# LPD-EPFL-ML/X-MAP

Measured on AMD Instinct MI355X. Metric: item_sim_pairs_per_s, higher is better.
Workload: dtype f64

## Files before the change

x-map_amd/csrc/common.h:

```cpp
#pragma once
#if defined(__HIP_DEVICE_COMPILE__) && !defined(__gfx950__)
#error "libxmap_hip is written for gfx950 (MI355X): build with --offload-arch=gfx950"
#endif
#include <hip/hip_runtime.h>
#include <stdint.h>
#include <stdio.h>
#include <string.h>

#include "../../include/xmap_hip.h"

namespace xmap {

void set_error(const char *fmt, ...);

#define XM_HIP(call)                                                                         \
    do {                                                                                     \
        hipError_t e_ = (call);                                                              \
        if (e_ != hipSuccess) {                                                              \
            xmap::set_error("%s:%d %s -> %s", __FILE__, __LINE__, #call, hipGetErrorString(e_)); \
            return XMAP_ERR_HIP;                                                             \
        }                                                                                    \
    } while (0)

#define XM_LAUNCH_CHECK() XM_HIP(hipGetLastError())

#define XM_ARG(cond)                                                        \
    do {                                                                    \
        if (!(cond)) {                                                      \
            xmap::set_error("%s:%d bad argument: %s", __FILE__, __LINE__, #cond); \
            return XMAP_ERR_ARG;                                            \
        }                                                                   \
    } while (0)

hipError_t xm_malloc_async(void **p, size_t bytes, hipStream_t st);
hipError_t xm_free_async(void *p, hipStream_t st);
struct XmScope {
    int dev; hipStream_t st; size_t live0; bool ok;
    explicit XmScope(hipStream_t st);
    ~XmScope();
    XmScope(const XmScope &) = delete;
    XmScope &operator=(const XmScope &) = delete;
};
#define XM_SCOPE(stream) xmap::XmScope xm_scope_((hipStream_t)(stream))
constexpr int HW_SLOTS = 2, HW_WORDS = 16;
constexpr int HW_PLAN = 0, HW_PAIRS = 1;
struct HostWait { int dev; int64_t *h; hipEvent_t ev[HW_SLOTS]; bool pending[HW_SLOTS]; };
HostWait *host_wait();
int host_wait_post(hipStream_t st, int slot, const void *d_src, int words);
int host_wait_take(int slot, const int64_t **h);
struct FillList {
    enum { MAX = 8 };
    void *p[MAX]; unsigned long long words[MAX]; unsigned val[MAX]; int n;
    FillList() : n(0) {}
    void add(void *ptr, size_t bytes, unsigned v = 0u) {
        if (n >= MAX) { n = MAX + 1; return; }
        p[n] = ptr; words[n] = bytes / 4; val[n] = v; n++;
    }
};
int fill_multi(hipStream_t st, const FillList &F);
int radix_sort_pairs(hipStream_t st, unsigned long long *keys, int *vals, unsigned long long *keys_tmp, int *vals_tmp, long long n,
                     int bits);

constexpr int WAVE = 64;

__device__ __forceinline__ int lane_id() { return threadIdx.x & 63; }

__device__ __forceinline__ int rl32(int v, int l) { return __builtin_amdgcn_readlane(v, l); }
__device__ __forceinline__ float rlf(float v, int l) { return __int_as_float(rl32(__float_as_int(v), l)); }
__device__ __forceinline__ long long rl64(long long v, int l) {
    int lo = rl32((int)(v & 0xffffffffll), l), hi = rl32((int)(v >> 32), l);
    return ((long long)hi << 32) | (unsigned int)lo;
}
__device__ __forceinline__ double rld(double v, int l) {
    return __longlong_as_double(rl64(__double_as_longlong(v), l));
}
__device__ __forceinline__ int uniform(int v) { return __builtin_amdgcn_readfirstlane(v); }

__device__ __forceinline__ unsigned long long lanemask_lt() {
    return (1ull << lane_id()) - 1ull;
}

__device__ __forceinline__ double wave_sum(double v) {
// ... 37 lines not shown
```

x-map_amd/csrc/tri.h:

```cpp
#pragma once
#include "common.h"
#include "tilesort.h"

namespace xmap {

constexpr int T_SLOTS = 1024;
constexpr int HMAX = 1024;
constexpr int SMALL_BOUND = 96;
constexpr int MID_BOUND = 384;

constexpr int N_CLASSES = 5;
constexpr int WIDE_MIN = 2048;
__host__ __device__ __forceinline__ int class_rank(int cls) {
    return cls == 4 ? 0 : (cls == 0 ? 1 : (cls == 2 ? 2 : (cls == 3 ? 3 : 4)));
}

__device__ __forceinline__ double weighted(double cs, int n, int cap) {
    const int mn = n < cap ? n : cap;
    return 1.0 * cs * (double)mn / (double)cap;
}
__device__ __forceinline__ unsigned long long ls_key(double d) {
    return (d != d) ? 0x7ff8000000000000ull : (unsigned long long)__double_as_longlong(d);
}

struct RaterRec { int e0; int pos_ge; float rating; int user; };
struct UbWide { int item_ge; int pad; double rating; };
struct RaterRecWide { int e0; int pos_ge; double rating; };

constexpr int COO_SHARDS = 4096;

int mirror_counts(hipStream_t st, int n_items, long long range_cap, int n_ranges, const unsigned long long *cur, const int *coo_i,
                  const int *coo_j, bool skip_self, int *part, int *counts, FillList *fills = nullptr);
void ts_geometry(int K, long long M, int ch, ts::Geo &G);
int ts_prepare(hipStream_t st, ts::Geo &G, const long long *ptr, FillList *fills = nullptr);
extern template __global__ void ts::k_ts_bin<3, true, ts::RecLoader<3>>(ts::Geo, ts::RecLoader<3>, long long, unsigned long long *__restrict__);

}
```

x-map_amd/csrc/tri_layout.hip:

```cpp
#include "tri.h"
#include "item_stats.h"

namespace xmap {

__device__ __forceinline__ unsigned long long wkey(int n, int item) {
    return ((unsigned long long)(unsigned)n << 32) | (unsigned)item;
}

constexpr int HIST_LDS = 2048;
constexpr int HIST_PER = 16;
__global__ __launch_bounds__(256) void k_hist(int I, const long long *iptr, int HB, int *hist) {
    __shared__ int loc[HIST_LDS];
    for (int t = threadIdx.x; t < HIST_LDS; t += 256) loc[t] = 0;
    __syncthreads();
    const long long base = (long long)blockIdx.x * 256 * HIST_PER;
    for (int q = 0; q < HIST_PER; q++) {
        const long long i = base + (long long)q * 256 + threadIdx.x;
        if (i < I) {
            long long n = iptr[i + 1] - iptr[i];
            int bin = n < HB - 1 ? (int)n : HB - 1;
            if (bin < HIST_LDS) atomicAdd(&loc[bin], 1); else atomicAdd(&hist[bin], 1);
        }
    }
    __syncthreads();
// ... 556 lines not shown
    for (long long p = p0 + lane_id(); p < p1; p += 64) {
        double r; int u;
        src.load(p, r, u);
        src.set_flag(p, r >= avg);
    }
}

__global__ __launch_bounds__(256) void k_rc_flags(long long nnz, RaterRec *rc, const int2 *ub, const double *info) {
    const long long p = (long long)blockIdx.x * blockDim.x + threadIdx.x;
    if (p >= nnz) return;
    const RaterRec r = rc[p];
    const int it = ub[(long long)r.e0 + (r.pos_ge & 0x7fffffff)].x & 0x7fffffff;
    if ((double)r.rating >= info[(size_t)it * 4]) rc[p].pos_ge = (int)((unsigned)r.pos_ge | 0x80000000u);
}

__global__ __launch_bounds__(256) void k_ub_flags(long long nnz, int2 *ub, const double *info) {
    const long long e = (long long)blockIdx.x * blockDim.x + threadIdx.x;
    if (e >= nnz) return;
    const int2 v = ub[e];
    if ((double)__int_as_float(v.y) >= info[(size_t)v.x * 4]) ub[e].x = (int)((unsigned)v.x | 0x80000000u);
}

}

using namespace xmap;

namespace {

void heavy_set_fills(FillList &F, int64_t n_users, int32_t *hist, int32_t *ctl) {
    F.add(hist, sizeof(int32_t) * (size_t)(n_users + 2));
    F.add(ctl, sizeof(int32_t), 0x7f7f7f7fu);
    F.add(ctl + 1, 3 * sizeof(int32_t));
}
int heavy_set(void *stream, int I, int64_t n_users, const int64_t *item_ptr, int32_t ch_min, int32_t *hist, int64_t *pre, int32_t *ctl,
              int32_t *hid, int32_t *hlist, bool filled = false) {
    hipStream_t st = (hipStream_t)stream;
    const int HB = (int)n_users + 2;
    if (!filled) {
        FillList F;
        heavy_set_fills(F, n_users, hist, ctl);
        int rc = fill_multi(st, F);
        if (rc) return rc;
    }
    if (I > 0) {
        k_hist<<<dim3((unsigned)((I + 256 * HIST_PER - 1) / (256 * HIST_PER))), dim3(256), 0, st>>>(I, (const long long *)item_ptr, HB, hist);
        XM_LAUNCH_CHECK();
    }
    int rcode = xmap_exclusive_scan_i32_to_i64(stream, hist, pre, HB, nullptr);
    if (rcode) return rcode;
    if (HB - 1 > ch_min) {
        k_threshold<<<dim3((unsigned)((HB + 255) / 256)), dim3(256), 0, st>>>(I, HB, (const long long *)pre, ch_min, ctl);
        XM_LAUNCH_CHECK();
    }
    if (I > 0) {
        k_mark_heavy<<<dim3((unsigned)((I + 255) / 256)), dim3(256), 0, st>>>(I, (const long long *)item_ptr, ctl, hid, hlist, ctl + 1);
        XM_LAUNCH_CHECK();
    }
    return XMAP_OK;
}

int read_heavy_ctl(hipStream_t st, const int32_t *ctl, int32_t *h_ctl) {
    XM_HIP(hipMemcpyAsync(h_ctl, ctl, 2 * sizeof(int32_t), hipMemcpyDeviceToHost, st));
    XM_HIP(hipStreamSynchronize(st));
    if (h_ctl[1] > HMAX) {
        set_error("heavy set larger than %d", HMAX);
        return XMAP_ERR_OVERFLOW;
    }
    return XMAP_OK;
}

int plan_rows(void *stream, const xmap_ratings *R, int32_t slot_target, const void *rc, const int64_t *pre, const int32_t *hid,
              const int32_t *ctl, int32_t *Q, int32_t *C, uint8_t *small, uint64_t *Wp, int32_t *Qcat, int64_t *uq_ptr, int64_t *uc_ptr,
              int32_t dups, int64_t *h_light, int64_t *h_heavy) {
    XM_ARG(slot_target > 0 && slot_target <= T_SLOTS);
    hipStream_t st = (hipStream_t)stream;
    const int I = R->n_items;
    if (I > 0) {
        k_plan2<<<dim3((unsigned)((I + 255) / 256)), dim3(256), 0, st>>>(
            I, (const long long *)R->item_ptr, (const RaterRec *)rc, (const long long *)pre, (int)R->n_users + 2, hid, ctl, slot_target, dups,
            Q, C, small, (unsigned long long *)Wp, Qcat);
        XM_LAUNCH_CHECK();
// ... 22 lines not shown
    return XMAP_OK;
}

template <typename Src>
int item_stats3(hipStream_t st, int I, int lo, int hi, const int64_t *item_ptr, const Src &src, double *info, double *norms,
                const BigList &B) {
    const long long *iptr = (const long long *)item_ptr;
    const dim3 grid((unsigned)((hi - lo + 15) / 16)), gridC((unsigned)((B.chunk_cap + 3) / 4)), gridI((unsigned)((B.item_cap + 63) / 64));
    k_item_stats3<Src><<<grid, dim3(256), 0, st>>>(I, lo, hi, iptr, src, info, norms, B);
    XM_LAUNCH_CHECK();
    k_item_chunks<Src><<<gridC, dim3(256), 0, st>>>(iptr, src, B);
    XM_LAUNCH_CHECK();
    k_item_big<<<gridI, dim3(64), 0, st>>>(I, B, info, norms);
    XM_LAUNCH_CHECK();
    if constexpr (Src::has_flags) {
        k_item_big_flags<Src><<<gridC, dim3(256), 0, st>>>(iptr, src, B, info);
        XM_LAUNCH_CHECK();
    }
    return XMAP_OK;
}

}

extern "C" {

int xmap_sim2_layout(void *stream, const xmap_ratings *R, const double *info, int32_t ch_min, int32_t *hist ,
                     int64_t *pre , int32_t *ctl , int32_t *hid, int32_t *hlist ,
                     uint64_t *ub_key , void *ub , void *rc ,
                     uint64_t *Wp , int32_t dups, int32_t *h_ctl ) {
    XM_ARG(R && info && hist && pre && ctl && hid && hlist && ub_key && ub && rc && Wp && ch_min >= 64);
    XM_ARG(R->nnz < 0x7fffffffLL && R->n_users < 0x7ffffff0LL);
    hipStream_t st = (hipStream_t)stream;
    const int I = R->n_items;
    int rcode = heavy_set(stream, I, R->n_users, R->item_ptr, ch_min, hist, pre, ctl, hid, hlist);
    if (rcode) return rcode;
    if (R->n_users > 0) {
        k_sort_profiles<<<dim3((unsigned)((R->n_users + 15) / 16)), dim3(256), 0, st>>>(
            R->n_users, (const long long *)R->user_ptr, R->user_item, R->user_rating, (const long long *)R->item_ptr, info,
            (unsigned long long *)ub_key, (int2 *)ub);
        XM_LAUNCH_CHECK();
    }
    XM_HIP(hipMemsetAsync(Wp, 0, sizeof(uint64_t) * (size_t)(I > 0 ? I : 1), st));
    if (R->nnz > 0) {
        if (dups) XM_HIP(hipMemsetAsync(ub_key, 0, sizeof(int32_t) * (size_t)R->nnz, st));
        k_rater_records<<<dim3((unsigned)((R->nnz + 255) / 256)), dim3(256), 0, st>>>(
            I, R->nnz, (const long long *)R->item_ptr, R->item_user, (const long long *)R->user_ptr, (const int2 *)ub,
            (RaterRec *)rc, dups ? (int *)ub_key : nullptr, (unsigned long long *)Wp);
        XM_LAUNCH_CHECK();
    }
    return h_ctl ? read_heavy_ctl(st, ctl, h_ctl) : XMAP_OK;
}

int xmap_sim2_plan(void *stream, const xmap_ratings *R, int32_t slot_target, const void *rc, const int64_t *pre,
                   const int32_t *hid, const int32_t *ctl, int32_t *Q, int32_t *C, uint8_t *small, uint64_t *Wp ,
                   int32_t *Qcat , int64_t *uq_ptr , int64_t *uc_ptr, int32_t dups,
                   int64_t *h_counts ) {
    XM_ARG(R && rc && Wp && pre && hid && ctl && Q && C && small && Qcat && uq_ptr && uc_ptr && h_counts);
    hipStream_t st = (hipStream_t)stream;
    const int I = R->n_items;
    int rcode = plan_rows(stream, R, slot_target, rc, pre, hid, ctl, Q, C, small, Wp, Qcat, uq_ptr, uc_ptr, dups, &h_counts[0], &h_counts[1]);
    if (rcode) return rcode;
    if (I > 0)
        XM_HIP(hipMemcpy2DAsync(&h_counts[2], sizeof(int64_t), uq_ptr, sizeof(int64_t) * (size_t)I, sizeof(int64_t),
                                N_CLASSES, hipMemcpyDeviceToHost, st));
    else
        for (int c = 0; c < N_CLASSES; c++) h_counts[2 + c] = 0;
    XM_HIP(hipStreamSynchronize(st));
// ... 60 lines not shown
    int rcode = xmap_sim3_plan_begin(stream, R, slot_target, pre, hid, ctl, Q, C, small, Wp, Qcat, uq_ptr, uc_ptr, dups, uq_item, uq_q, uc_item,
                                     uc_c, cap_light, cap_heavy);
    if (rcode) return rcode;
    return xmap_sim3_plan_wait(cap_light, cap_heavy, h_out);
}

int xmap_sim3_layout(void *stream, const xmap_ratings *R, int64_t *item_ptr, const double *rating64, int32_t ch_min, int32_t phases,
                     int32_t stats_lo, int32_t stats_hi, int32_t *cnt, double *u_avg, double *u_norm, int32_t *hist, int64_t *pre, int32_t *ctl, int32_t *hid, int32_t *hlist,
                     uint64_t *ub_key, void *ub, void *srec, void *bufA, void *bufB, void *rc, uint64_t *Wp, double *info,
                     double *norms, int32_t *h_ctl) {
    XM_SCOPE(stream);
    XM_ARG(R && item_ptr && (const int64_t *)item_ptr == R->item_ptr && cnt && u_avg && hist && pre && ctl && hid && hlist);
    XM_ARG(ub_key && ub && srec && bufA && bufB && rc && Wp && info && norms && ch_min >= 64);
    XM_ARG(R->nnz < 0x7fffffffLL && R->n_users < 0x7ffffff0LL && R->n_items >= 0);
    XM_ARG(rating64 || u_norm);
    XM_ARG(stats_lo >= 0 && stats_lo <= stats_hi && stats_hi <= R->n_items && (phases & ~XMAP_LAYOUT_ALL) == 0);
    hipStream_t st = (hipStream_t)stream;
    const int I = R->n_items;
    const long long nnz = R->nnz;
    const bool wide = rating64 != nullptr;
    const size_t In = (size_t)(I > 0 ? I : 1);
    int rcode = XMAP_OK;
    const bool stats = (phases & XMAP_LAYOUT_STATS) && stats_hi > stats_lo;
    BigList B;
    bool b_cleared = false;
    if (stats) {
        B.chunk_cap = nnz / STAT_CHK + nnz / STAT_BIG + 2;
        B.item_cap = nnz / STAT_BIG + 2;
        XM_HIP(xm_malloc_async((void **)&B.counters, 2 * sizeof(unsigned), st));
        XM_HIP(xm_malloc_async((void **)&B.chunks, sizeof(int2) * (size_t)B.chunk_cap, st));
        XM_HIP(xm_malloc_async((void **)&B.items, sizeof(int4) * (size_t)B.item_cap, st));
        XM_HIP(xm_malloc_async((void **)&B.part, sizeof(double) * ITEM_PART * (size_t)B.chunk_cap, st));
    }
    if (phases & XMAP_LAYOUT_RECORDS) {
        FillList F;
        F.add(cnt, sizeof(int32_t) * In);
        heavy_set_fills(F, R->n_users, hist, ctl);
        F.add(Wp, sizeof(uint64_t) * In);
        if (stats) { F.add(B.counters, 2 * sizeof(unsigned)); b_cleared = true; }
        const char *cb_env = getenv("XMAP_COUNT_PART_MIN");
        const long long cb_min = cb_env ? atoll(cb_env) : 2000000ll;
        if (nnz >= cb_min && I > 0) {
            rcode = mirror_counts(st, I, nnz, 1, nullptr, nullptr, R->user_item, false, (int *)bufA, cnt, &F);
            if (rcode) return rcode;
        } else {
            rcode = fill_multi(st, F);
            if (rcode) return rcode;
            if (nnz > 0) {
                k_count3<<<dim3((unsigned)((nnz + CNT_CHUNK - 1) / CNT_CHUNK)), dim3(256), 0, st>>>(nnz, R->user_item, cnt);
                XM_LAUNCH_CHECK();
            }
        }
        rcode = xmap_exclusive_scan_i32_to_i64(stream, cnt, item_ptr, I, nullptr);
        if (rcode) return rcode;
        if (!wide) {
            rcode = xmap_user_stats(stream, R, u_avg, u_norm);
            if (rcode) return rcode;
        }
        rcode = heavy_set(stream, I, R->n_users, item_ptr, ch_min, hist, pre, ctl, hid, hlist, true);
        if (rcode) return rcode;
        if (R->n_users > 0 && nnz > 0) {
            const dim3 grid((unsigned)((R->n_users + 15) / 16));
            (wide ? k_sort_profiles3<true> : k_sort_profiles3<false>)<<<grid, dim3(256), 0, st>>>(
                R->n_users, (const long long *)R->user_ptr, R->user_item, wide ? nullptr : R->user_rating, rating64, cnt,
                (unsigned long long *)ub_key, ub, (unsigned long long *)srec);
            XM_LAUNCH_CHECK();
        }
        if (nnz > 0 && I > 0) {
            ts::Geo G;
            ts_geometry(I, nnz, wide ? ts::Chunk<3>::CH : ts::Chunk<2>::CH, G);
            rcode = ts_prepare(st, G, (const long long *)item_ptr);
            if (rcode) return rcode;
            rcode = wide ? sort_rater_records<3>(st, G, nnz, srec, bufA, bufB, R->user_ptr, rc, Wp)
                         : sort_rater_records<2>(st, G, nnz, srec, bufA, bufB, R->user_ptr, rc, Wp);
            if (rcode) return rcode;
        }
    }
    if (stats) {
        if (!b_cleared) XM_HIP(hipMemsetAsync(B.counters, 0, 2 * sizeof(unsigned), st));
        rcode = wide ? item_stats3(st, I, stats_lo, stats_hi, item_ptr, RcWideSrc{(const RaterRecWide *)rc}, info, norms, B)
                     : item_stats3(st, I, stats_lo, stats_hi, item_ptr, RcSrc{(RaterRec *)rc, u_avg}, info, norms, B);
        if (rcode) return rcode;
    }
    if (!wide && nnz > 0 && I > 0) {
        if (phases & XMAP_LAYOUT_RC_FLAGS) {
            k_rc_flags<<<dim3((unsigned)((nnz + 255) / 256)), dim3(256), 0, st>>>(nnz, (RaterRec *)rc, (const int2 *)ub, info);
            XM_LAUNCH_CHECK();
        }
        if (phases & XMAP_LAYOUT_UB_FLAGS) {
            k_ub_flags<<<dim3((unsigned)((nnz + 255) / 256)), dim3(256), 0, st>>>(nnz, (int2 *)ub, info);
            XM_LAUNCH_CHECK();
        }
    }
    return h_ctl ? read_heavy_ctl(st, ctl, h_ctl) : XMAP_OK;
}
}
```

x-map_amd/csrc/tri_mirror.hip:

```cpp
#include "tri.h"

namespace xmap {

constexpr int SC_U = 4;
__global__ __launch_bounds__(256) void k_scatter(long long n, const int *coo_i, const int *coo_j, const double *coo_sim,
                                                 const int *coo_mutu, const int *coo_nij, const double *coo_aux,
                                                 const long long *row_ptr, int *fill, int *col, double *sim, int *mutu,
                                                 int *nij, double *aux) {
    const int lane = lane_id();
    const long long r0 = ((long long)blockIdx.x * (blockDim.x >> 6) + uniform((int)(threadIdx.x >> 6))) * (64 * SC_U) + lane;
    int i[SC_U], j[SC_U], m[SC_U], nn[SC_U];
    double s[SC_U], x[SC_U];
    bool valid[SC_U];
#pragma unroll
    for (int u = 0; u < SC_U; u++) {
        const long long r = r0 + 64 * u;
        i[u] = (r < n) ? coo_i[r] : -1;
    }
#pragma unroll
    for (int u = 0; u < SC_U; u++) {
        const long long r = r0 + 64 * u;
        valid[u] = i[u] >= 0;
        j[u] = 0; m[u] = 0; nn[u] = 0; s[u] = 0.0; x[u] = 0.0;
        if (valid[u]) {
// ... 370 lines not shown
    const int nch = (int)((size + G.ch - 1) / G.ch);
    if (nch == 0) return;
    const unsigned base = atomicAdd(&G.counters[0], (unsigned)nch);
    for (int x = 0; x < nch; x++)
        if ((long long)base + x < G.clist_cap) G.clist[base + x] = make_int2(a, x);
}

}

template __global__ void ts::k_ts_bin<3, true, ts::RecLoader<3>>(ts::Geo, ts::RecLoader<3>, long long, unsigned long long *__restrict__);

void ts_geometry(int K, long long M, int ch, ts::Geo &G) {
    G.K = K; G.M = M; G.ch = ch;
    G.ts_log = 11;
    for (;;) {
        const long long TS = 1ll << G.ts_log;
        long long kw = M / (4 * (long long)(K > 0 ? K : 1));
        const long long kw_min = TS / (ts::NK_MAX - 2) + 1;
        if (kw < kw_min) kw = kw_min;
        if (kw < 4) kw = 4;
        const long long tiles = ((M + (long long)K * kw) >> G.ts_log) + 1;
        if (tiles <= (long long)ts::NA_MAX * ts::NB || G.ts_log >= 30) {
            G.KW = (int)kw;
            G.NA = (int)((tiles + ts::NB - 1) / ts::NB);
            if (G.NA < 1) G.NA = 1;
            if (G.NA > ts::NA_MAX) G.NA = ts::NA_MAX;
            G.T = G.NA * ts::NB;
            return;
        }
        G.ts_log++;
    }
}

int ts_prepare(hipStream_t st, ts::Geo &G, const long long *ptr, FillList *fills) {
    G.ptr = ptr;
    G.clist_cap = G.M / G.ch + G.NA + 1;
    G.slist_cap = G.M / ts::SL + (G.M >> G.ts_log) + 2;
    XM_HIP(xm_malloc_async((void **)&G.tile_key0, sizeof(int) * ((size_t)G.T + 1), st));
    XM_HIP(xm_malloc_async((void **)&G.tile_pos0, sizeof(long long) * ((size_t)G.T + 1), st));
    XM_HIP(xm_malloc_async((void **)&G.tile_large, sizeof(int) * (size_t)G.T, st));
    unsigned long long *z = nullptr;
    const size_t nz = (size_t)G.NA + 2 * (size_t)G.T + 1;
    XM_HIP(xm_malloc_async((void **)&z, sizeof(unsigned long long) * nz, st));
    G.curA = z; G.curB = z + G.NA; G.counters = (unsigned *)(z + G.NA + 2 * (size_t)G.T);
    XM_HIP(xm_malloc_async((void **)&G.clist, sizeof(int2) * (size_t)G.clist_cap, st));
    XM_HIP(xm_malloc_async((void **)&G.slist, sizeof(int2) * (size_t)G.slist_cap, st));
    FillList own;
    FillList &F = fills ? *fills : own;
    F.add(z, sizeof(unsigned long long) * nz);
    F.add(G.tile_large, sizeof(int) * (size_t)G.T, 0xffffffffu);
    int rcode = fill_multi(st, F);
    if (rcode) return rcode;
    ts::k_ts_plan<<<dim3((unsigned)((G.K + 255) / 256)), dim3(256), 0, st>>>(G);
    XM_LAUNCH_CHECK();
    ts::k_ts_chunks<<<dim3((unsigned)((G.NA + 255) / 256)), dim3(256), 0, st>>>(G);
    XM_LAUNCH_CHECK();
    return XMAP_OK;
}

namespace {
template <bool AUX, bool SHARE>
int mirror_levels(hipStream_t st, const ts::Geo &G, int64_t coo_cap, const int32_t *coo_i, const int32_t *coo_j, const double *coo_sim,
                  const int32_t *coo_mutu, const int32_t *coo_nij, const double *coo_aux, const longlong2 *chunks, const unsigned *n_chunks,
                  long long chunk_cap, int64_t n_pairs, const int32_t *own, const int64_t *row_ptr, int32_t *fill, void *bufA, void *bufB,
                  int32_t *col, double *sim, int32_t *mutu, int32_t *nij, double *aux, int row_lo, int row_hi) {
    constexpr int RW = AUX ? 4 : 3;
    CooLoaderT<AUX, SHARE> LA{coo_i, coo_j, coo_sim, coo_mutu, coo_nij, coo_aux, chunks, n_chunks, (const long long *)row_ptr, fill,
                              col, sim, mutu, nij, aux, row_lo, row_hi};
    ts::RecLoader<RW> LB{(const unsigned long long *)bufA};
    ts::k_ts_bin<RW, false, CooLoaderT<AUX, SHARE>><<<dim3((unsigned)chunk_cap), dim3(ts::BT), 0, st>>>(G, LA, coo_cap, (unsigned long long *)bufA);
    XM_LAUNCH_CHECK();
    ts::k_ts_bin<RW, true, ts::RecLoader<RW>><<<dim3((unsigned)G.clist_cap), dim3(ts::BT), 0, st>>>(G, LB, n_pairs, (unsigned long long *)bufB);
    XM_LAUNCH_CHECK();
    k_mir_tiles<AUX><<<dim3((unsigned)G.T), dim3(ts::CT), 0, st>>>(G, (const unsigned long long *)bufB, (const long long *)row_ptr, own, col,
                                                                   sim, mutu, nij, aux);
    XM_LAUNCH_CHECK();
    k_mir_large<AUX><<<dim3((unsigned)G.slist_cap), dim3(ts::LT), 0, st>>>(G, (const unsigned long long *)bufB, (const long long *)row_ptr, own,
                                                                            col, sim, mutu, nij, aux);
    XM_LAUNCH_CHECK();
    return XMAP_OK;
}
}

int mirror_counts(hipStream_t st, int n_items, long long range_cap, int n_ranges, const unsigned long long *cur, const int *coo_i,
                  const int *coo_j, bool skip_self, int *part, int *counts, FillList *fills) {
    FillList own;
    FillList &F = fills ? *fills : own;
    if (n_items <= 0 || range_cap <= 0 || n_ranges <= 0) return fill_multi(st, F);
// ... 58 lines not shown
    return mirror_counts(st, n_items, d_shards ? coo_cap / COO_SHARDS : n_pairs, d_shards ? COO_SHARDS : 1,
                         (const unsigned long long *)d_shards, coo_i, coo_j, skip_self != 0, (int *)scratch, mir, &F);
}

int xmap_sim3_mirror(void *stream, int32_t n_items, int64_t coo_cap, const int32_t *coo_i, const int32_t *coo_j,
                     const double *coo_sim, const int32_t *coo_mutu, const int32_t *coo_nij, const int64_t *d_shards, int64_t n_pairs,
                     const int32_t *own, const int32_t *mir, int32_t *tot, int64_t *row_ptr, int64_t *mptr, int32_t *fill,
                     void *bufA, void *bufB, int32_t *col, double *sim, int32_t *mutu, int32_t *nij, const double *coo_aux, double *aux,
                     int32_t row_lo, int32_t row_hi) {
    XM_SCOPE(stream);
    XM_ARG(row_lo >= 0 && row_lo <= row_hi && row_hi <= n_items);
    XM_ARG(coo_i && coo_j && coo_sim && coo_mutu && coo_nij && own && mir && tot && row_ptr && mptr && fill && bufA && bufB);
    XM_ARG(col && sim && mutu && nij && n_items >= 0 && coo_cap >= 0 && n_pairs >= 0 && n_pairs < 0x7fffffffLL);
    XM_ARG(d_shards ? (coo_cap >= COO_SHARDS) : (n_pairs <= coo_cap));
    XM_ARG((coo_aux != nullptr) == (aux != nullptr));
    hipStream_t st = (hipStream_t)stream;
    const int I = n_items;
    int rcode = xmap_exclusive_scan2_i32_to_i64(stream, own, mir, 1, row_ptr, mptr, I, nullptr);
    if (rcode) return rcode;
    if (n_pairs == 0 || I == 0 || coo_cap == 0) return XMAP_OK;
    ts::Geo G;
    ts_geometry(I, n_pairs, coo_aux ? ts::Chunk<4>::CH : ts::Chunk<3>::CH, G);
    static_assert(ts::Chunk<3>::CH <= ts::Chunk<4>::CH && ts::Chunk<4>::CH % ts::Chunk<3>::CH == 0, "chunk lists by the narrow record width");
    const int n_shards = d_shards ? COO_SHARDS : 1;
    const long long shard_cap = d_shards ? coo_cap / COO_SHARDS : coo_cap;
    const long long chunk_cap = n_pairs / ts::Chunk<3>::CH + n_shards + 1;
    longlong2 *chunks = nullptr;
    unsigned *n_chunks = nullptr;
    XM_HIP(xm_malloc_async((void **)&chunks, sizeof(longlong2) * (size_t)chunk_cap, st));
    XM_HIP(xm_malloc_async((void **)&n_chunks, sizeof(unsigned), st));
    FillList F;
    F.add(fill, sizeof(int32_t) * (size_t)I);
    F.add(n_chunks, sizeof(unsigned));
    rcode = ts_prepare(st, G, (const long long *)mptr, &F);
    if (rcode) return rcode;
    k_coo_chunks<<<dim3((unsigned)((n_shards + 255) / 256)), dim3(256), 0, st>>>(n_shards, shard_cap, (const unsigned long long *)d_shards,
                                                                                 n_pairs, chunks, n_chunks, chunk_cap);
    XM_LAUNCH_CHECK();
    const bool share = row_lo > 0 || row_hi < I;
    auto levels = coo_aux ? (share ? mirror_levels<true, true> : mirror_levels<true, false>)
                          : (share ? mirror_levels<false, true> : mirror_levels<false, false>);
    return levels(st, G, coo_cap, coo_i, coo_j, coo_sim, coo_mutu, coo_nij, coo_aux, chunks, n_chunks, chunk_cap, n_pairs, own, row_ptr, fill,
                  bufA, bufB, col, sim, mutu, nij, aux, row_lo, row_hi);
}
}
```

x-map_amd/csrc/tri_pairs.hip:

```cpp
#include <type_traits>

#include "tri.h"

namespace xmap {

constexpr uint32_t T_EMPTY = 0xFFFFFFFFu;

struct TriArgs {
    const long long *iptr;
    const RaterRec *rc;
    const int2 *ub;
    const double *u_avg; const double *nrm;
    int cap;
    const int *Q; const uint8_t *small; const int *uq_item; const int *uq_q; long long unit_lo, unit_hi;
    const int *hid; const int *hlist; const int *CH; const int *uc_item; const int *uc_c;
    const long long *uc_ptr; const int *C;
    double *hp_hi; double *hp_lo; int *hp_cnt; int *hp_mut;
    long long shard_cap;
    unsigned long long *shard_cur;
    unsigned long long *shard_occ;
    int *coo_i; int *coo_j; double *coo_sim; int *coo_mutu; int *coo_nij;
    double *coo_aux;
    int *rowcnt;
    int *mircnt;
// ... 460 lines not shown
                hi += A.hp_hi[o];
            } else {
                dd_add(hi, lo, A.hp_hi[o]);
                dd_add(hi, lo, A.hp_lo[o]);
            }
        }
        cnt[s] = cn; mut[s] = mu; dot[s] = hi;
    }
    if (nc == 0) return;
    __syncthreads();
    const int w = uniform((int)(threadIdx.x >> 6));
    append_pairs(A, i, w * (HMAX / 4), (w + 1) * (HMAX / 4),
        [&](int s, int &j, int &n, int &m, double &sv, bool &o) {
            o = cnt[s] != 0;
            if (!o) return false;
            j = A.hlist[s]; n = (int)cnt[s]; m = (int)mut[s];
            return finish_pair<METHOD>(A, i, j, n, m, dot[s], sv);
        },
        [&](int s, bool o, bool keep, double sv) {
            if (o) { if (keep) dot[s] = sv; else cnt[s] = 0; }
        },
        [&](int s, int &j, int &n, int &m, double &sv) {
            if (cnt[s] == 0) return false;
            j = A.hlist[s]; n = (int)cnt[s]; m = (int)mut[s]; sv = dot[s];
            return true;
        },
        [&](int s) { return 0.0; });
}

}

using namespace xmap;

struct SideStreams { hipStream_t s[N_CLASSES + 1]; hipEvent_t fork, done[N_CLASSES + 1]; int dev; };
static SideStreams *side_streams() {
    static thread_local SideStreams *cur[64] = {nullptr};
    int dev = 0;
    if (hipGetDevice(&dev) != hipSuccess || dev < 0 || dev >= 64) { set_error("hipGetDevice failed"); return nullptr; }
    if (cur[dev]) return cur[dev];
    SideStreams *p = new SideStreams();
    p->dev = dev;
    bool ok = hipEventCreateWithFlags(&p->fork, hipEventDisableTiming) == hipSuccess;
    for (int c = 0; c <= N_CLASSES && ok; c++)
        ok = hipStreamCreateWithFlags(&p->s[c], hipStreamNonBlocking) == hipSuccess &&
             hipEventCreateWithFlags(&p->done[c], hipEventDisableTiming) == hipSuccess;
    if (!ok) { set_error("could not create the side streams"); delete p; return nullptr; }
    cur[dev] = p;
    return p;
}

namespace {

template <int METHOD, bool LS>
int launch_tri(int c, dim3 grid, hipStream_t st, const TriArgs &A) {
#define XM_TRI(LOG_SLOTS, NW) k_pair_tri<METHOD, LOG_SLOTS, NW, LS><<<grid, dim3(64 * NW), 0, st>>>(A)
    switch (c) {
    case 0: XM_TRI(10, 16); break;
    case 1: XM_TRI(10, 4); break;
    case 2: XM_TRI(9, 2); break;
    case 3: XM_TRI(8, 1); break;
    default: XM_TRI(7, 1); break;
    }
#undef XM_TRI
    XM_LAUNCH_CHECK();
    return XMAP_OK;
}

int launch_heavy(int method, hipStream_t st, const TriArgs &A, int n_units, int n_heavy) {
    const bool cos = method == XMAP_COSINE;
    if (n_units > 0) {
        (cos ? k_pair_heavy<XMAP_COSINE> : k_pair_heavy<XMAP_ADJUST_COSINE>)<<<dim3((unsigned)n_units), dim3(64 * HEAVY_WAVES), 0, st>>>(A);
        XM_LAUNCH_CHECK();
    }
    if (n_heavy > 0) {
        (cos ? k_heavy_merge<XMAP_COSINE> : k_heavy_merge<XMAP_ADJUST_COSINE>)<<<dim3((unsigned)n_heavy), dim3(256), 0, st>>>(A, n_heavy);
        XM_LAUNCH_CHECK();
    }
    return XMAP_OK;
}

}

// ... 129 lines not shown
```

x-map_amd/csrc/util.hip:

```cpp
#include <stdarg.h>
#include <stdlib.h>
#include <vector>

#include "common.h"

namespace xmap {
static thread_local char g_err[512] = "";
void set_error(const char *fmt, ...) {
    va_list ap;
    va_start(ap, fmt);
    vsnprintf(g_err, sizeof(g_err), fmt, ap);
    va_end(ap);
}

namespace {
struct Chunk { char *base; size_t size, used; };
struct Arena { int dev; hipStream_t st; std::vector<Chunk> chunks; size_t live; };
thread_local std::vector<Arena> g_arenas;
constexpr size_t ARENA_KEEP = (size_t)256 << 20;
Arena *arena_find(int dev, hipStream_t st) {
    for (Arena &a : g_arenas) if (a.dev == dev && a.st == st) return &a;
    return nullptr;
}
Arena *arena_of(hipStream_t st) {
// ... 75 lines not shown
    if (!ok) { set_error("could not create the pinned read-back block"); delete p; return nullptr; }
    cur[dev] = p;
    return p;
}
int host_wait_post(hipStream_t st, int slot, const void *d_src, int words) {
    XM_ARG(slot >= 0 && slot < HW_SLOTS && words >= 0 && words <= HW_WORDS);
    HostWait *w = host_wait();
    if (!w) return XMAP_ERR_HIP;
    if (w->pending[slot]) {
        XM_HIP(hipEventSynchronize(w->ev[slot]));
        w->pending[slot] = false;
    }
    int64_t *h = w->h + (size_t)slot * HW_WORDS;
    for (int x = 0; x < HW_WORDS; x++) h[x] = 0;
    if (words) XM_HIP(hipMemcpyAsync(h, d_src, sizeof(int64_t) * (size_t)words, hipMemcpyDeviceToHost, st));
    XM_HIP(hipEventRecord(w->ev[slot], st));
    w->pending[slot] = true;
    return XMAP_OK;
}
int host_wait_take(int slot, const int64_t **h) {
    XM_ARG(slot >= 0 && slot < HW_SLOTS && h);
    HostWait *w = host_wait();
    if (!w) return XMAP_ERR_HIP;
    if (!w->pending[slot]) {
        set_error("read-back slot %d waited for without a post", slot);
        return XMAP_ERR_ARG;
    }
    w->pending[slot] = false;
    XM_HIP(hipEventSynchronize(w->ev[slot]));
    *h = w->h + (size_t)slot * HW_WORDS;
    return XMAP_OK;
}

__global__ __launch_bounds__(256) void k_fill_multi(FillList F) {
    const int y = blockIdx.y;
    unsigned *p = (unsigned *)F.p[y];
    const unsigned long long n = F.words[y];
    const unsigned v = F.val[y];
    for (unsigned long long i = (unsigned long long)blockIdx.x * 256 + threadIdx.x; i < n; i += (unsigned long long)gridDim.x * 256) p[i] = v;
}
int fill_multi(hipStream_t st, const FillList &F) {
    XM_ARG(F.n >= 0 && F.n <= FillList::MAX);
    unsigned long long most = 0;
    for (int y = 0; y < F.n; y++) most = F.words[y] > most ? F.words[y] : most;
    if (F.n == 0 || most == 0) return XMAP_OK;
    unsigned long long bx = (most + 1023) / 1024;
    if (bx > 2048) bx = 2048;
    k_fill_multi<<<dim3((unsigned)bx, (unsigned)F.n), dim3(256), 0, st>>>(F);
    XM_LAUNCH_CHECK();
    return XMAP_OK;
}

constexpr int SCAN_THREADS = 256;
constexpr int SCAN_ITEMS = 8;
constexpr int SCAN_TILE = SCAN_THREADS * SCAN_ITEMS;
constexpr int SCAN2_MAX_TILES = 2048;

__device__ __forceinline__ long long block_exclusive_scan(long long v, long long *total, long long *smem) {
    int lane = threadIdx.x & 63, w = threadIdx.x >> 6;
    long long inc = v;
#pragma unroll
    for (int d = 1; d < 64; d <<= 1) {
        long long o = __shfl_up(inc, d, 64);
        if (lane >= d) inc += o;
    }
    if (lane == 63) smem[w] = inc;
// ... 54 lines not shown
__global__ __launch_bounds__(SCAN_THREADS) void k_tile_scan(ScanIn<TIn> S, long long n, long long n_tiles, const long long *tile_sum,
                                                            long long *out0, long long *out1) {
    __shared__ long long smem[4];
    const int y = blockIdx.y;
    tile_sum += (long long)y * n_tiles;
    long long *out = y ? out1 : out0;
    long long off;
    if (SELF) {
        long long part = 0;
        for (long long t = threadIdx.x; t < (long long)blockIdx.x; t += SCAN_THREADS) part += tile_sum[t];
        block_exclusive_scan(part, &off, smem);
    } else {
        off = tile_sum[blockIdx.x];
    }
    long long base = (long long)blockIdx.x * SCAN_TILE + (long long)threadIdx.x * SCAN_ITEMS;
    long long v[SCAN_ITEMS];
    long long s = 0;
#pragma unroll
    for (int k = 0; k < SCAN_ITEMS; k++) {
        v[k] = (base + k < n) ? S.load(y, base + k) : 0;
        s += v[k];
    }
    long long tot;
    long long ex = block_exclusive_scan(s, &tot, smem) + off;
#pragma unroll
    for (int k = 0; k < SCAN_ITEMS; k++) {
        if (base + k < n) out[base + k] = ex;
        ex += v[k];
    }
    if (SELF && blockIdx.x == gridDim.x - 1 && threadIdx.x == 0) out[n] = off + tot;
}

template <typename TIn>
static int exclusive_scan(hipStream_t st, int n_arrays, const TIn *in0, const TIn *in1, int plus, int64_t *out0, int64_t *out1, int64_t n,
                          int64_t *h_total) {
    XM_ARG(n >= 0 && (n_arrays == 1 || n_arrays == 2));
    XM_SCOPE(st);
    const int64_t n_tiles = (n + SCAN_TILE - 1) / SCAN_TILE;
    XM_ARG(n_tiles < 0x7fffffffLL);
    const ScanIn<TIn> S{in0, in1, plus};
    if (n_tiles == 0) {
        XM_HIP(hipMemsetAsync(out0 + n, 0, sizeof(int64_t), st));
        if (n_arrays == 2) XM_HIP(hipMemsetAsync(out1 + n, 0, sizeof(int64_t), st));
    } else {
        long long *tile = nullptr;
        XM_HIP(xm_malloc_async((void **)&tile, sizeof(long long) * (size_t)n_tiles * (size_t)n_arrays, st));
        const dim3 grid((unsigned)n_tiles, (unsigned)n_arrays);
        k_tile_sums<TIn><<<grid, dim3(SCAN_THREADS), 0, st>>>(S, n, n_tiles, tile);
        XM_LAUNCH_CHECK();
        if (n_tiles <= SCAN2_MAX_TILES) {
            k_tile_scan<TIn, true><<<grid, dim3(SCAN_THREADS), 0, st>>>(S, n, n_tiles, tile, (long long *)out0, (long long *)out1);
            XM_LAUNCH_CHECK();
        } else {
            k_scan_tile_sums<<<dim3(1, (unsigned)n_arrays), dim3(SCAN_THREADS), 0, st>>>(tile, n_tiles, (long long *)(out0 + n),
                                                                                          (long long *)(out1 ? out1 + n : nullptr));
            XM_LAUNCH_CHECK();
            k_tile_scan<TIn, false><<<grid, dim3(SCAN_THREADS), 0, st>>>(S, n, n_tiles, tile, (long long *)out0, (long long *)out1);
            XM_LAUNCH_CHECK();
        }
        XM_HIP(xm_free_async(tile, st));
    }
    if (h_total) {
        XM_HIP(hipMemcpyAsync(h_total, out0 + n, sizeof(int64_t), hipMemcpyDeviceToHost, st));
        if (n_arrays == 2) XM_HIP(hipMemcpyAsync(h_total + 1, out1 + n, sizeof(int64_t), hipMemcpyDeviceToHost, st));
        XM_HIP(hipStreamSynchronize(st));
    }
    return XMAP_OK;
}
}

extern "C" {
const char *xmap_last_error(void) { return xmap::g_err; }
int xmap_version(void) { return 114; }

int xmap_trim(void) {
    XM_HIP(hipDeviceSynchronize());
    int dev = 0;
    XM_HIP(hipGetDevice(&dev));
    for (xmap::Arena &a : xmap::g_arenas) {
        if (a.dev != dev || a.live != 0) continue;
        for (xmap::Chunk &c : a.chunks) (void)hipFree(c.base);
        a.chunks.clear();
    }
    return XMAP_OK;
}

int xmap_debug_arena(void *stream, int64_t *live, int64_t *reserved) {
    XM_ARG(live && reserved);
    int dev = 0;
    XM_HIP(hipGetDevice(&dev));
    *live = 0; *reserved = 0;
    if (xmap::Arena *a = xmap::arena_find(dev, (hipStream_t)stream)) {
        *live = (int64_t)a->live;
        for (xmap::Chunk &c : a->chunks) *reserved += (int64_t)c.size;
    }
    return XMAP_OK;
}
int xmap_debug_arena_call(void *stream, int64_t bytes, int fail) {
    using namespace xmap;
    XM_SCOPE(stream);
    hipStream_t st = (hipStream_t)stream;
    void *a = nullptr, *b = nullptr;
    XM_HIP(xm_malloc_async(&a, (size_t)bytes, st));
    XM_HIP(xm_malloc_async(&b, 1024, st));
    XM_ARG(!fail);
    XM_HIP(xm_free_async(b, st));
    XM_HIP(xm_free_async(a, st));
    return XMAP_OK;
}

int xmap_exclusive_scan_i64(void *stream, const int64_t *in, int64_t *out, int64_t n, int64_t *h_total) {
    XM_ARG(out && (in || n == 0));
    return xmap::exclusive_scan<long long>((hipStream_t)stream, 1, (const long long *)in, nullptr, 0, out, nullptr, n, h_total);
}
int xmap_exclusive_scan_i32_to_i64(void *stream, const int32_t *in, int64_t *out, int64_t n, int64_t *h_total) {
    XM_ARG(out && (in || n == 0));
    return xmap::exclusive_scan<int>((hipStream_t)stream, 1, in, nullptr, 0, out, nullptr, n, h_total);
}
int xmap_exclusive_scan2_i32_to_i64(void *stream, const int32_t *in_a, const int32_t *in_b, int32_t a_plus_b, int64_t *out_a,
                                    int64_t *out_b, int64_t n, int64_t *h_totals) {
    XM_ARG(out_a && out_b && ((in_a && in_b) || n == 0));
    return xmap::exclusive_scan<int>((hipStream_t)stream, 2, in_a, in_b, a_plus_b ? 1 : 0, out_a, out_b, n, h_totals);
}
int xmap_scan_self_tiles(void) { return xmap::SCAN2_MAX_TILES; }
}
```

Baseline: 25.51 billion.

## Overlap profile sorting with layout table builds on a side stream

```diff
diff --git a/x-map_amd/csrc/common.h b/x-map_amd/csrc/common.h
--- a/x-map_amd/csrc/common.h
+++ b/x-map_amd/csrc/common.h
@@ -48,6 +48,31 @@
 HostWait *host_wait();
 int host_wait_post(hipStream_t st, int slot, const void *d_src, int words);
 int host_wait_take(int slot, const int64_t **h);
+constexpr int SIDE_STREAMS = 6;
+constexpr int SIDE_LAYOUT = SIDE_STREAMS - 1;
+struct SideStreams { hipStream_t s[SIDE_STREAMS]; hipEvent_t fork, done[SIDE_STREAMS]; int dev; };
+SideStreams *side_streams();
+bool stage_a_serial();
+struct Fork {
+    hipStream_t st, s; hipEvent_t done; bool open;
+    Fork() : st(nullptr), s(nullptr), done(nullptr), open(false) {}
+    ~Fork() { if (open) (void)join(); }
+    Fork(const Fork &) = delete;
+    Fork &operator=(const Fork &) = delete;
+    int begin(hipStream_t caller, SideStreams *side, int k, hipEvent_t after) {
+        XM_HIP(hipStreamWaitEvent(side->s[k], after, 0));
+        st = caller; s = side->s[k]; done = side->done[k]; open = true;
+        return XMAP_OK;
+    }
+    int join() {
+        if (!open) return XMAP_OK;
+        open = false;
+        XM_HIP(hipEventRecord(done, s));
+        XM_HIP(hipStreamWaitEvent(st, done, 0));
+        return XMAP_OK;
+    }
+};
+int scan_i32_to_i64_on(hipStream_t arena, hipStream_t run, const int32_t *in, int64_t *out, int64_t n);
 struct FillList {
     enum { MAX = 8 };
     void *p[MAX]; unsigned long long words[MAX]; unsigned val[MAX]; int n;
diff --git a/x-map_amd/csrc/tri.h b/x-map_amd/csrc/tri.h
--- a/x-map_amd/csrc/tri.h
+++ b/x-map_amd/csrc/tri.h
@@ -32,7 +32,7 @@
 int mirror_counts(hipStream_t st, int n_items, long long range_cap, int n_ranges, const unsigned long long *cur, const int *coo_i,
                   const int *coo_j, bool skip_self, int *part, int *counts, FillList *fills = nullptr);
 void ts_geometry(int K, long long M, int ch, ts::Geo &G);
-int ts_prepare(hipStream_t st, ts::Geo &G, const long long *ptr, FillList *fills = nullptr);
+int ts_prepare(hipStream_t st, hipStream_t run, ts::Geo &G, const long long *ptr, FillList *fills = nullptr);
 extern template __global__ void ts::k_ts_bin<3, true, ts::RecLoader<3>>(ts::Geo, ts::RecLoader<3>, long long, unsigned long long *__restrict__);
 
 }
diff --git a/x-map_amd/csrc/tri_layout.hip b/x-map_amd/csrc/tri_layout.hip
--- a/x-map_amd/csrc/tri_layout.hip
+++ b/x-map_amd/csrc/tri_layout.hip
@@ -612,9 +612,8 @@
     F.add(ctl, sizeof(int32_t), 0x7f7f7f7fu);
     F.add(ctl + 1, 3 * sizeof(int32_t));
 }
-int heavy_set(void *stream, int I, int64_t n_users, const int64_t *item_ptr, int32_t ch_min, int32_t *hist, int64_t *pre, int32_t *ctl,
-              int32_t *hid, int32_t *hlist, bool filled = false) {
-    hipStream_t st = (hipStream_t)stream;
+int heavy_set(hipStream_t arena, hipStream_t st, int I, int64_t n_users, const int64_t *item_ptr, int32_t ch_min, int32_t *hist, int64_t *pre,
+              int32_t *ctl, int32_t *hid, int32_t *hlist, bool filled = false) {
     const int HB = (int)n_users + 2;
     if (!filled) {
         FillList F;
@@ -626,7 +625,7 @@
         k_hist<<<dim3((unsigned)((I + 256 * HIST_PER - 1) / (256 * HIST_PER))), dim3(256), 0, st>>>(I, (const long long *)item_ptr, HB, hist);
         XM_LAUNCH_CHECK();
     }
-    int rcode = xmap_exclusive_scan_i32_to_i64(stream, hist, pre, HB, nullptr);
+    int rcode = scan_i32_to_i64_on(arena, st, hist, pre, HB);
     if (rcode) return rcode;
     if (HB - 1 > ch_min) {
         k_threshold<<<dim3((unsigned)((HB + 255) / 256)), dim3(256), 0, st>>>(I, HB, (const long long *)pre, ch_min, ctl);
@@ -715,7 +714,7 @@
     XM_ARG(R->nnz < 0x7fffffffLL && R->n_users < 0x7ffffff0LL);
     hipStream_t st = (hipStream_t)stream;
     const int I = R->n_items;
-    int rcode = heavy_set(stream, I, R->n_users, R->item_ptr, ch_min, hist, pre, ctl, hid, hlist);
+    int rcode = heavy_set(st, st, I, R->n_users, R->item_ptr, ch_min, hist, pre, ctl, hid, hlist);
     if (rcode) return rcode;
     if (R->n_users > 0) {
         k_sort_profiles<<<dim3((unsigned)((R->n_users + 15) / 16)), dim3(256), 0, st>>>(
@@ -842,7 +841,13 @@
         XM_HIP(xm_malloc_async((void **)&B.items, sizeof(int4) * (size_t)B.item_cap, st));
         XM_HIP(xm_malloc_async((void **)&B.part, sizeof(double) * ITEM_PART * (size_t)B.chunk_cap, st));
     }
+    Fork tables;
     if (phases & XMAP_LAYOUT_RECORDS) {
+        SideStreams *side = nullptr;
+        if (!stage_a_serial()) {
+            side = side_streams();
+            if (!side) return XMAP_ERR_HIP;
+        }
         FillList F;
         F.add(cnt, sizeof(int32_t) * In);
         heavy_set_fills(F, R->n_users, hist, ctl);
@@ -861,30 +866,50 @@
                 XM_LAUNCH_CHECK();
             }
         }
-        rcode = xmap_exclusive_scan_i32_to_i64(stream, cnt, item_ptr, I, nullptr);
+        auto sort_profiles = [&]() -> int {
+            if (R->n_users > 0 && nnz > 0) {
+                const dim3 grid((unsigned)((R->n_users + 15) / 16));
+                (wide ? k_sort_profiles3<true> : k_sort_profiles3<false>)<<<grid, dim3(256), 0, st>>>(
+                    R->n_users, (const long long *)R->user_ptr, R->user_item, wide ? nullptr : R->user_rating, rating64, cnt,
+                    (unsigned long long *)ub_key, ub, (unsigned long long *)srec);
+                XM_LAUNCH_CHECK();
+            }
+            return XMAP_OK;
+        };
+        hipStream_t tb = st;
+        if (side) {
+            XM_HIP(hipEventRecord(side->fork, st));
+            rcode = tables.begin(st, side, SIDE_LAYOUT, side->fork);
+            if (rcode) return rcode;
+            tb = tables.s;
+            rcode = sort_profiles();
+            if (rcode) return rcode;
+        }
+        rcode = scan_i32_to_i64_on(st, tb, cnt, item_ptr, I);
         if (rcode) return rcode;
         if (!wide) {
-            rcode = xmap_user_stats(stream, R, u_avg, u_norm);
+            rcode = xmap_user_stats(tb, R, u_avg, u_norm);
             if (rcode) return rcode;
         }
-        rcode = heavy_set(stream, I, R->n_users, item_ptr, ch_min, hist, pre, ctl, hid, hlist, true);
+        rcode = heavy_set(st, tb, I, R->n_users, item_ptr, ch_min, hist, pre, ctl, hid, hlist, true);
         if (rcode) return rcode;
-        if (R->n_users > 0 && nnz > 0) {
-            const dim3 grid((unsigned)((R->n_users + 15) / 16));
-            (wide ? k_sort_profiles3<true> : k_sort_profiles3<false>)<<<grid, dim3(256), 0, st>>>(
-                R->n_users, (const long long *)R->user_ptr, R->user_item, wide ? nullptr : R->user_rating, rating64, cnt,
-                (unsigned long long *)ub_key, ub, (unsigned long long *)srec);
-            XM_LAUNCH_CHECK();
+        if (!side) {
+            rcode = sort_profiles();
+            if (rcode) return rcode;
         }
         if (nnz > 0 && I > 0) {
             ts::Geo G;
             ts_geometry(I, nnz, wide ? ts::Chunk<3>::CH : ts::Chunk<2>::CH, G);
-            rcode = ts_prepare(st, G, (const long long *)item_ptr);
+            rcode = ts_prepare(st, tb, G, (const long long *)item_ptr);
+            if (rcode) return rcode;
+            rcode = tables.join();
             if (rcode) return rcode;
             rcode = wide ? sort_rater_records<3>(st, G, nnz, srec, bufA, bufB, R->user_ptr, rc, Wp)
                          : sort_rater_records<2>(st, G, nnz, srec, bufA, bufB, R->user_ptr, rc, Wp);
             if (rcode) return rcode;
         }
+        rcode = tables.join();
+        if (rcode) return rcode;
     }
     if (stats) {
         if (!b_cleared) XM_HIP(hipMemsetAsync(B.counters, 0, 2 * sizeof(unsigned), st));
diff --git a/x-map_amd/csrc/tri_mirror.hip b/x-map_amd/csrc/tri_mirror.hip
--- a/x-map_amd/csrc/tri_mirror.hip
+++ b/x-map_amd/csrc/tri_mirror.hip
@@ -426,7 +426,7 @@
     }
 }
 
-int ts_prepare(hipStream_t st, ts::Geo &G, const long long *ptr, FillList *fills) {
+int ts_prepare(hipStream_t st, hipStream_t run, ts::Geo &G, const long long *ptr, FillList *fills) {
     G.ptr = ptr;
     G.clist_cap = G.M / G.ch + G.NA + 1;
     G.slist_cap = G.M / ts::SL + (G.M >> G.ts_log) + 2;
@@ -443,11 +443,11 @@
     FillList &F = fills ? *fills : own;
     F.add(z, sizeof(unsigned long long) * nz);
     F.add(G.tile_large, sizeof(int) * (size_t)G.T, 0xffffffffu);
-    int rcode = fill_multi(st, F);
+    int rcode = fill_multi(run, F);
     if (rcode) return rcode;
-    ts::k_ts_plan<<<dim3((unsigned)((G.K + 255) / 256)), dim3(256), 0, st>>>(G);
-    XM_LAUNCH_CHECK();
-    ts::k_ts_chunks<<<dim3((unsigned)((G.NA + 255) / 256)), dim3(256), 0, st>>>(G);
+    ts::k_ts_plan<<<dim3((unsigned)((G.K + 255) / 256)), dim3(256), 0, run>>>(G);
+    XM_LAUNCH_CHECK();
+    ts::k_ts_chunks<<<dim3((unsigned)((G.NA + 255) / 256)), dim3(256), 0, run>>>(G);
     XM_LAUNCH_CHECK();
     return XMAP_OK;
 }
@@ -572,7 +572,7 @@
     FillList F;
     F.add(fill, sizeof(int32_t) * (size_t)I);
     F.add(n_chunks, sizeof(unsigned));
-    rcode = ts_prepare(st, G, (const long long *)mptr, &F);
+    rcode = ts_prepare(st, st, G, (const long long *)mptr, &F);
     if (rcode) return rcode;
     k_coo_chunks<<<dim3((unsigned)((n_shards + 255) / 256)), dim3(256), 0, st>>>(n_shards, shard_cap, (const unsigned long long *)d_shards,
                                                                                  n_pairs, chunks, n_chunks, chunk_cap);
diff --git a/x-map_amd/csrc/tri_pairs.hip b/x-map_amd/csrc/tri_pairs.hip
--- a/x-map_amd/csrc/tri_pairs.hip
+++ b/x-map_amd/csrc/tri_pairs.hip
@@ -516,22 +516,7 @@
 
 using namespace xmap;
 
-struct SideStreams { hipStream_t s[N_CLASSES + 1]; hipEvent_t fork, done[N_CLASSES + 1]; int dev; };
-static SideStreams *side_streams() {
-    static thread_local SideStreams *cur[64] = {nullptr};
-    int dev = 0;
-    if (hipGetDevice(&dev) != hipSuccess || dev < 0 || dev >= 64) { set_error("hipGetDevice failed"); return nullptr; }
-    if (cur[dev]) return cur[dev];
-    SideStreams *p = new SideStreams();
-    p->dev = dev;
-    bool ok = hipEventCreateWithFlags(&p->fork, hipEventDisableTiming) == hipSuccess;
-    for (int c = 0; c <= N_CLASSES && ok; c++)
-        ok = hipStreamCreateWithFlags(&p->s[c], hipStreamNonBlocking) == hipSuccess &&
-             hipEventCreateWithFlags(&p->done[c], hipEventDisableTiming) == hipSuccess;
-    if (!ok) { set_error("could not create the side streams"); delete p; return nullptr; }
-    cur[dev] = p;
-    return p;
-}
+static_assert(SIDE_STREAMS == N_CLASSES + 1, "one side stream per table class and one for the heavy rows");
 
 namespace {
 
diff --git a/x-map_amd/csrc/util.hip b/x-map_amd/csrc/util.hip
--- a/x-map_amd/csrc/util.hip
+++ b/x-map_amd/csrc/util.hip
@@ -131,6 +131,26 @@
     return XMAP_OK;
 }
 
+SideStreams *side_streams() {
+    static thread_local SideStreams *cur[64] = {nullptr};
+    int dev = 0;
+    if (hipGetDevice(&dev) != hipSuccess || dev < 0 || dev >= 64) { set_error("hipGetDevice failed"); return nullptr; }
+    if (cur[dev]) return cur[dev];
+    SideStreams *p = new SideStreams();
+    p->dev = dev;
+    bool ok = hipEventCreateWithFlags(&p->fork, hipEventDisableTiming) == hipSuccess;
+    for (int c = 0; c < SIDE_STREAMS && ok; c++)
+        ok = hipStreamCreateWithFlags(&p->s[c], hipStreamNonBlocking) == hipSuccess &&
+             hipEventCreateWithFlags(&p->done[c], hipEventDisableTiming) == hipSuccess;
+    if (!ok) { set_error("could not create the side streams"); delete p; return nullptr; }
+    cur[dev] = p;
+    return p;
+}
+bool stage_a_serial() {
+    const char *e = getenv("XMAP_STAGE_A_SERIAL");
+    return e && atoi(e) == 1;
+}
+
 __global__ __launch_bounds__(256) void k_fill_multi(FillList F) {
     const int y = blockIdx.y;
     unsigned *p = (unsigned *)F.p[y];
@@ -251,10 +271,10 @@
 }
 
 template <typename TIn>
-static int exclusive_scan(hipStream_t st, int n_arrays, const TIn *in0, const TIn *in1, int plus, int64_t *out0, int64_t *out1, int64_t n,
+static int exclusive_scan(hipStream_t arena, hipStream_t st, int n_arrays, const TIn *in0, const TIn *in1, int plus, int64_t *out0, int64_t *out1, int64_t n,
                           int64_t *h_total) {
     XM_ARG(n >= 0 && (n_arrays == 1 || n_arrays == 2));
-    XM_SCOPE(st);
+    XM_SCOPE(arena);
     const int64_t n_tiles = (n + SCAN_TILE - 1) / SCAN_TILE;
     XM_ARG(n_tiles < 0x7fffffffLL);
     const ScanIn<TIn> S{in0, in1, plus};
@@ -263,7 +283,7 @@
         if (n_arrays == 2) XM_HIP(hipMemsetAsync(out1 + n, 0, sizeof(int64_t), st));
     } else {
         long long *tile = nullptr;
-        XM_HIP(xm_malloc_async((void **)&tile, sizeof(long long) * (size_t)n_tiles * (size_t)n_arrays, st));
+        XM_HIP(xm_malloc_async((void **)&tile, sizeof(long long) * (size_t)n_tiles * (size_t)n_arrays, arena));
         const dim3 grid((unsigned)n_tiles, (unsigned)n_arrays);
         k_tile_sums<TIn><<<grid, dim3(SCAN_THREADS), 0, st>>>(S, n, n_tiles, tile);
         XM_LAUNCH_CHECK();
@@ -277,7 +297,7 @@
             k_tile_scan<TIn, false><<<grid, dim3(SCAN_THREADS), 0, st>>>(S, n, n_tiles, tile, (long long *)out0, (long long *)out1);
             XM_LAUNCH_CHECK();
         }
-        XM_HIP(xm_free_async(tile, st));
+        XM_HIP(xm_free_async(tile, arena));
     }
     if (h_total) {
         XM_HIP(hipMemcpyAsync(h_total, out0 + n, sizeof(int64_t), hipMemcpyDeviceToHost, st));
@@ -286,11 +306,15 @@
     }
     return XMAP_OK;
 }
+int scan_i32_to_i64_on(hipStream_t arena, hipStream_t run, const int32_t *in, int64_t *out, int64_t n) {
+    XM_ARG(out && (in || n == 0));
+    return exclusive_scan<int>(arena, run, 1, in, nullptr, 0, out, nullptr, n, nullptr);
+}
 }
 
 extern "C" {
 const char *xmap_last_error(void) { return xmap::g_err; }
-int xmap_version(void) { return 114; }
+int xmap_version(void) { return 115; }
 
 int xmap_trim(void) {
     XM_HIP(hipDeviceSynchronize());
@@ -330,16 +354,16 @@
 
 int xmap_exclusive_scan_i64(void *stream, const int64_t *in, int64_t *out, int64_t n, int64_t *h_total) {
     XM_ARG(out && (in || n == 0));
-    return xmap::exclusive_scan<long long>((hipStream_t)stream, 1, (const long long *)in, nullptr, 0, out, nullptr, n, h_total);
+    return xmap::exclusive_scan<long long>((hipStream_t)stream, (hipStream_t)stream, 1, (const long long *)in, nullptr, 0, out, nullptr, n, h_total);
 }
 int xmap_exclusive_scan_i32_to_i64(void *stream, const int32_t *in, int64_t *out, int64_t n, int64_t *h_total) {
     XM_ARG(out && (in || n == 0));
-    return xmap::exclusive_scan<int>((hipStream_t)stream, 1, in, nullptr, 0, out, nullptr, n, h_total);
+    return xmap::exclusive_scan<int>((hipStream_t)stream, (hipStream_t)stream, 1, in, nullptr, 0, out, nullptr, n, h_total);
 }
 int xmap_exclusive_scan2_i32_to_i64(void *stream, const int32_t *in_a, const int32_t *in_b, int32_t a_plus_b, int64_t *out_a,
                                     int64_t *out_b, int64_t n, int64_t *h_totals) {
     XM_ARG(out_a && out_b && ((in_a && in_b) || n == 0));
-    return xmap::exclusive_scan<int>((hipStream_t)stream, 2, in_a, in_b, a_plus_b ? 1 : 0, out_a, out_b, n, h_totals);
+    return xmap::exclusive_scan<int>((hipStream_t)stream, (hipStream_t)stream, 2, in_a, in_b, a_plus_b ? 1 : 0, out_a, out_b, n, h_totals);
 }
 int xmap_scan_self_tiles(void) { return xmap::SCAN2_MAX_TILES; }
 }
```

New measurement: 26.10 billion (median of 6 runs). 2.3% higher.
